# seceq/zkir

Hardware: AMD Instinct MI355X
Metric: trace rows/sec (2^20-cycle fib: execution-trace fill + BabyBear NTT/LDE + Poseidon2 Merkle commitment) (higher is better)
Workload: dtype u32 (Baby Bear, 31-bit modular) / u64 trace words

## Files before the change

### include/zkir_amd_experimental.h

```cpp
#ifndef ZKIR_AMD_EXPERIMENTAL_H
#define ZKIR_AMD_EXPERIMENTAL_H
#include "zkir_amd.h"
#ifdef __cplusplus
extern "C" {
#endif

double zkir_modmul_peak_per_s(void* hip_stream);
double zkir_hbm_copy_peak_gbs(uint64_t bytes, void* hip_stream);
int zkir_commit_fused01_launch(const zkir_stark_ctx* ctx, const zkir_trace_columns* trace, uint64_t n_real, uint32_t* m, uint32_t width, uint32_t* out, void* hip_stream);
int zkir_ntt_strided_variant_launch(const zkir_stark_ctx* ctx, uint32_t* data, uint32_t width, int variant, int forward, void* hip_stream);

int zkir_commit_overlapped_launch(const zkir_stark_ctx* ctx, uint32_t* in, uint32_t width, uint32_t* out, uint32_t* tree, uint32_t group, void* hip_stream);

int zkir_lowdeg_prove_stages(zkir_stark_ctx* ctx, const uint32_t* lde_mat, uint32_t width, const uint32_t* tree, uint32_t num_queries, uint32_t pow_bits, uint32_t* proof_host,
                             uint64_t cap_words, uint64_t* n_words, float stage_ms[4], void* hip_stream);
int zkir_lowdeg_combine_launch(const zkir_stark_ctx* ctx, const uint32_t* lde_mat, uint32_t width, const uint32_t gamma[4], uint32_t* gpow_scratch, uint32_t* cw, void* hip_stream);

int zkir_eval_prove_stages(zkir_stark_ctx* ctx, const uint32_t* lde_mat, uint32_t width, const uint32_t* tree, const uint32_t* points, uint32_t n_points, uint32_t num_queries,
                           uint32_t pow_bits, uint32_t* proof_host, uint64_t cap_words, uint64_t* n_words, float stage_ms[6], void* hip_stream);
uint64_t zkir_eval_at_scratch_words(uint32_t log_n, uint32_t width, uint32_t n_points);
int zkir_eval_at_launch(const zkir_stark_ctx* ctx, const uint32_t* lde_mat, uint32_t width, const uint32_t* points, uint32_t n_points, uint32_t* scratch, uint32_t* evals, void* hip_stream);
uint64_t zkir_eval_quotient_scratch_words(uint32_t log_m, uint32_t width, uint32_t n_points);
int zkir_eval_quotient_launch(const zkir_stark_ctx* ctx, const uint32_t* lde_mat, uint32_t width, const uint32_t gamma[4], const uint32_t* points, uint32_t n_points,
                              const uint32_t* evals, uint32_t* scratch, uint32_t* cw, void* hip_stream);
// ... 16 lines not shown
int zkir_pcs_verify_last_stage_ms(double ms[3]);
int zkir_verify_queries_last_stage_ms(double ms[3]);
int zkir_stark_query_stage_probe(const uint32_t* proof, uint64_t proof_words, uint32_t what, uint32_t index, int device, void* hip_stream);
int zkir_verify_many_memory_host(const uint32_t* const* proofs, const uint64_t* proof_words, const zkir_public_inputs* const* expects, uint32_t n, int32_t* verdicts);
int zkir_verify_rate_many_memory_host(const uint32_t* const* proofs, const uint64_t* proof_words, const zkir_public_inputs* const* expects, const uint32_t* min_queries,
                                      const uint32_t* min_pow_bits, uint32_t n, int32_t* verdicts);
int zkir_mem_sections_stage_host(const uint32_t* const* secs, const uint64_t* n_words, const uint32_t* modes, const uint64_t* code_words, const uint8_t* const* blobs, const size_t* blob_lens,
                                 const uint32_t* alphas, const uint32_t* lambdas, uint32_t n, int32_t* verdicts, uint32_t* digests, uint32_t* sums);
int zkir_mem_sections_stage_launch(const uint32_t* const* secs, const uint64_t* n_words, const uint32_t* modes, const uint64_t* code_words, const uint8_t* const* blobs, const size_t* blob_lens,
                                   const uint32_t* alphas, const uint32_t* lambdas, uint32_t n, int32_t* verdicts, uint32_t* digests, uint32_t* sums, void* hip_stream);
int zkir_verify_many_memory_probe(const uint32_t* const* proofs, const uint64_t* proof_words, const zkir_public_inputs* const* expects, uint32_t n, int32_t* verdicts, uint32_t what,
                                  uint32_t index, int device, void* hip_stream);
int zkir_verify_many_tapes_host(const uint32_t* const* proofs, const uint64_t* proof_words, const zkir_public_inputs* const* expects, uint32_t n, int32_t* verdicts);
int zkir_verify_rate_many_tapes_host(const uint32_t* const* proofs, const uint64_t* proof_words, const zkir_public_inputs* const* expects, const uint32_t* min_queries,
                                     const uint32_t* min_pow_bits, uint32_t n, int32_t* verdicts);
int zkir_tape_sections_stage_host(const uint32_t* const* hash_secs, const uint64_t* hash_words, const uint32_t* const* wide_secs, const uint64_t* wide_words, const uint64_t* n_real,
                                  const uint64_t* code_end, const uint32_t* alphas, const uint32_t* lambdas, uint32_t n, int32_t* hash_verdicts, int32_t* wide_verdicts, uint32_t* digests,
                                  uint32_t* sums);
int zkir_tape_sections_stage_launch(const uint32_t* const* hash_secs, const uint64_t* hash_words, const uint32_t* const* wide_secs, const uint64_t* wide_words, const uint64_t* n_real,
                                    const uint64_t* code_end, const uint32_t* alphas, const uint32_t* lambdas, uint32_t n, int32_t* hash_verdicts, int32_t* wide_verdicts, uint32_t* digests,
                                    uint32_t* sums, void* hip_stream);
int zkir_verify_many_tapes_probe(const uint32_t* const* proofs, const uint64_t* proof_words, const zkir_public_inputs* const* expects, uint32_t n, int32_t* verdicts, uint32_t what,
                                 uint32_t index, int device, void* hip_stream);

#ifdef __cplusplus
}
#endif
#endif
```

### zkir_amd/csrc/poseidon2.h

```cpp
#pragma once
#include "babybear.h"

#ifndef P2_RF_UNROLL
#define P2_RF_UNROLL 1
#endif
namespace p2 {

constexpr int T = 12, RF = 8, RP = 22, RATE = 8, DIGEST = 4;

struct Consts {
  uint32_t ext[RF][T];
  uint32_t in[RP];
  uint32_t diag[T];
  uint32_t pre[RF][T];
  uint32_t ext0_s[T];
  uint64_t pre_b[RF][T];
  uint32_t in_scale;
  uint32_t out_scale;
  uint32_t carry;
  int32_t in0_neg;
  int32_t pr_c[RP];
  uint64_t pr_a[RP];
  uint64_t pr_k[T];
};

inline uint64_t splitmix64(uint64_t& s) {
  uint64_t z = (s += 0x9E3779B97F4A7C15ull);
  z = (z ^ (z >> 30)) * 0xBF58476D1CE4E5B9ull;
  z = (z ^ (z >> 27)) * 0x94D049BB133111EBull;
  return z ^ (z >> 31);
}

inline void ext_matrix_inverse(uint32_t inv[T][T]) {
  static const uint32_t M4[4][4] = {{5, 7, 1, 3}, {4, 6, 1, 1}, {1, 3, 5, 7}, {1, 1, 4, 6}};
  uint32_t a[T][2 * T];
  for (int i = 0; i < T; i++)
    for (int j = 0; j < T; j++) {
      a[i][j] = M4[i & 3][j & 3] * ((i >> 2) == (j >> 2) ? 2u : 1u);
      a[i][T + j] = i == j;
    }
  for (int col = 0; col < T; col++) {
    int piv = col;
    while (a[piv][col] == 0) piv++;
    for (int j = 0; j < 2 * T; j++) { const uint32_t t = a[col][j]; a[col][j] = a[piv][j]; a[piv][j] = t; }
    const uint32_t pinv = bb::inv(a[col][col]);
    for (int j = 0; j < 2 * T; j++) a[col][j] = bb::mul(a[col][j], pinv);
    for (int i = 0; i < T; i++) {
      if (i == col || a[i][col] == 0) continue;
      const uint32_t f = a[i][col];
      for (int j = 0; j < 2 * T; j++) a[i][j] = bb::sub(a[i][j], bb::mul(f, a[col][j]));
    }
  }
  for (int i = 0; i < T; i++) for (int j = 0; j < T; j++) inv[i][j] = a[i][T + j];
}

inline void generate(Consts& c) {
  uint64_t s = 0x5A4B49522D50322Dull;
  auto next = [&]() -> uint32_t { for (;;) { const uint32_t v = (uint32_t)(splitmix64(s) >> 33); if (v < bb::P) return bb::to_mont(v); } };
  for (int r = 0; r < RF; r++) for (int i = 0; i < T; i++) c.ext[r][i] = next();
  for (int r = 0; r < RP; r++) c.in[r] = next();
  c.diag[0] = bb::to_mont(bb::P - 2);
  for (int i = 1; i < T; i++) c.diag[i] = bb::to_mont(1u << (i - 1));
  uint32_t minv[T][T];
  ext_matrix_inverse(minv);
  for (int r = 0; r < RF; r++)
    for (int i = 0; i < T; i++) {
      uint32_t v = 0;
      if (r != RF / 2 - 1 && r != RF - 1)
        for (int j = 0; j < T; j++) v = bb::add(v, bb::mul(minv[i][j], bb::from_mont(c.ext[r + 1][j])));
      c.pre[r][i] = bb::to_mont(bb::to_mont(v));
    }
  {
    constexpr uint64_t INV7 = 1725656503ull;
    const uint32_t R = bb::R1, Rinv = bb::inv(R);
    const uint32_t R6 = bb::pow(R, 6);
    uint32_t g[RF + 1], h[RF];
    g[RF / 2] = R;
    for (int r = RF / 2 - 1; r >= 0; r--) { h[r] = bb::mul(g[r + 1], R); g[r] = bb::pow(bb::mul(h[r], R6), INV7); }
    {
      uint32_t f[RP], hx[RP];
      for (int r = 0; r < RP; r++) { f[r] = r < 3 ? R : bb::mul(f[r - 3], Rinv); hx[r] = bb::pow(bb::mul(f[r], R6), INV7); }
      const uint32_t G = bb::mul(f[RP - 1], Rinv), R2c = bb::mul(R, R);
      for (int r = 0; r < RP; r++) {
        const uint32_t hn = r + 1 < RP ? hx[r + 1] : G, rcn = bb::from_mont(r + 1 < RP ? c.in[r + 1] : c.ext[RF / 2][0]);
        c.pr_c[r] = (int32_t)bb::mul(bb::mul(hn, R2c), bb::inv(f[r]));
        c.pr_a[r] = bb::mul(bb::mul(hn, rcn), R);
      }
      c.pr_k[0] = 0;
      for (int i = 1; i < T; i++) c.pr_k[i] = bb::mul(f[RP - 1], bb::from_mont(c.ext[RF / 2][i]));
      g[RF / 2] = G;
    }
    for (int r = RF / 2; r < RF; r++) { h[r] = bb::mul(bb::pow(g[r], 7), bb::inv(R6)); g[r + 1] = bb::mul(h[r], Rinv); }
    const uint32_t f_in = bb::mul(g[0], R), f_out = g[RF];
    for (int i = 0; i < T; i++) c.ext0_s[i] = bb::mul(bb::from_mont(c.ext[0][i]), f_in);
    for (int r = 0; r < RF; r++)
      for (int i = 0; i < T; i++) {
        uint32_t v = 0;
        if (r != RF / 2 - 1 && r != RF - 1)
          for (int j = 0; j < T; j++) v = bb::add(v, bb::mul(minv[i][j], bb::from_mont(c.ext[r + 1][j])));
        c.pre_b[r][i] = ((uint64_t)bb::P << 32) | bb::mul(bb::mul(v, h[r]), R);
      }
    c.in_scale = bb::mul(f_in, R);
    c.out_scale = bb::mul(R, bb::inv(f_out));
    c.carry = bb::mul(bb::mul(f_in, R), bb::inv(f_out));
// ... 114 lines not shown
  uint64_t acc = (uint64_t)w[1];
#pragma unroll
  for (int i = 2; i < T; i++) acc += (uint64_t)w[i];
  const int64_t sum = bb::sacc_add((int64_t)acc, s0);
  x = int_next_x(smad<-2>(sum, s0), c, r);
#pragma unroll
  for (int i = 1; i < T; i++) w[i] = (int64_t)(((uint64_t)w[i] << (i - 1)) + (uint64_t)sum);
}
constexpr uint64_t lazy_rounds_bound(uint64_t start, int rounds) {
  uint64_t b[T] = {}, top = 0;
  for (int i = 1; i < T; i++) b[i] = start;
  for (int r = 0; r < rounds; r++) {
    uint64_t sum = bb::P;
    for (int i = 1; i < T; i++) sum += b[i];
    if (sum + 2 * (uint64_t)bb::P > top) top = sum + 2 * (uint64_t)bb::P;
    for (int i = 1; i < T; i++) { b[i] = sum + (b[i] << (i - 1)); if (b[i] > top) top = b[i]; }
  }
  return top;
}
constexpr uint64_t lazy_reduced_bound(uint64_t acc) { return (acc >> 32) + bb::P / 2 + 2; }
static_assert(lazy_rounds_bound(1ull << 31, 3) < (1ull << 62), "three partial rounds on words below 2^31 stay inside what a Montgomery reduction takes");
static_assert(lazy_reduced_bound(lazy_rounds_bound(1ull << 31, 3)) <= (1ull << 31), ".. and their reduction is a word below 2^31 again");
static_assert(lazy_reduced_bound(lazy_rounds_bound(1ull << 31, 1) + bb::P) < bb::P, "the words leave the last round (one round + the next full round's constant) inside (-p, p)");
BB_HD void int_rounds_scaled(uint32_t* s, const Consts& c) {
  int32_t x = (int32_t)s[0] + c.in0_neg;
  int32_t t[T];
  int64_t w[T];
#pragma unroll
  for (int i = 1; i < T; i++) t[i] = (int32_t)s[i];
#pragma unroll 1
  for (int r = 0; r < RP - 1; r += 3) {
    int_round_a(x, t, w, c, r);
    int_round_w(x, w, c, r + 1);
    int_round_w(x, w, c, r + 2);
#pragma unroll
    for (int i = 1; i < T; i++) t[i] = bb::smont_reduce_wide(w[i]);
  }
  int_round_a(x, t, w, c, RP - 1);
  s[0] = (uint32_t)x;
#pragma unroll
  for (int i = 1; i < T; i++) s[i] = (uint32_t)bb::smont_reduce_wide((int64_t)((uint64_t)w[i] + c.pr_k[i]));
}
BB_HD void permute_scaled(uint32_t* s, const Consts& c) {
  ext_linear_scaled<true>(s, c.ext0_s);
#pragma unroll P2_RF_UNROLL
  for (int r = 0; r < RF / 2; r++) {
#pragma unroll
    for (int i = 0; i < T; i++) s[i] = sbox_biased(s[i], c.pre_b[r][i]);
    ext_linear_scaled<false>(s, nullptr);
  }
  int_rounds_scaled(s, c);
#pragma unroll P2_RF_UNROLL
  for (int r = RF / 2; r < RF; r++) {
#pragma unroll
    for (int i = 0; i < T; i++) s[i] = sbox_biased(s[i], c.pre_b[r][i]);
    ext_linear_scaled<false>(s, nullptr);
  }
}

#if defined(__HIPCC__)
template <int CTRL>
__device__ __forceinline__ uint32_t quad_perm(uint32_t v) { return (uint32_t)__builtin_amdgcn_mov_dpp((int)v, CTRL, 0xF, 0xF, true); }
template <int CTRL>
__device__ __forceinline__ uint64_t quad_perm64(uint64_t v) { return ((uint64_t)quad_perm<CTRL>((uint32_t)(v >> 32)) << 32) | quad_perm<CTRL>((uint32_t)v); }

template <bool ADD_RC>
__device__ __forceinline__ void ext_linear_quad_scaled(uint32_t* s, const uint32_t* m4row, const uint32_t* rc) {
  uint64_t y[3];
#pragma unroll
  for (int b = 0; b < 3; b++) {
    const uint32_t v0 = quad_perm<0x00>(s[b]), v1 = quad_perm<0x55>(s[b]), v2 = quad_perm<0xAA>(s[b]), v3 = quad_perm<0xFF>(s[b]);
    y[b] = (uint64_t)v0 * m4row[0] + (uint64_t)v1 * m4row[1] + (uint64_t)v2 * m4row[2] + (uint64_t)v3 * m4row[3];
  }
  const uint64_t sum = y[0] + y[1] + y[2];
#pragma unroll
  for (int b = 0; b < 3; b++) {
    uint64_t v = y[b] + sum;
    if (ADD_RC) v += rc[b];
    s[b] = bb::mont_reduce_wide(v);
  }
// ... 108 lines not shown
```

### zkir_amd/csrc/stark.hip

```cpp
#include <hip/hip_runtime.h>

#include <array>
#include <atomic>
#include <chrono>
#include <cstdio>
#include <cstdlib>
#include <cstddef>
#include <memory>
#include <mutex>
#include <vector>

#include "../../include/zkir_amd.h"
#include "../../include/zkir_amd_experimental.h"
#include "air.h"
#include "babybear.h"
#include "fri_shape.h"
#include "host.h"
#include "hashcall.h"
#include "poseidon2.h"
#include "verify_stages.h"

namespace {

constexpr int NT = 256;
// ... 414 lines not shown
}


__global__ __launch_bounds__(NT) void selector_inverse_kernel(uint32_t log_m, const uint32_t* __restrict__ tw_fwd, uint32_t* __restrict__ inv_xm1) {
  const uint32_t N2 = 1u << log_m, N = N2 >> 1;
  const uint32_t j0 = (blockIdx.x * NT + threadIdx.x) * 8;
  if (j0 >= N2) return;
  uint32_t d[8], pre[8];
  uint32_t run = bb::R1;
#pragma unroll
  for (int k = 0; k < 8; k++) {
    const uint32_t j = j0 + k;
    const uint32_t wj = j < N ? tw_fwd[j] : bb::neg(tw_fwd[j - N]);
    d[k] = bb::sub(bb::mont_mul(wj, bb::to_mont(bb::GEN)), bb::R1);
    pre[k] = run; run = bb::mont_mul(run, d[k]);
  }
  uint32_t inv = bb::R1, b = run, e = bb::P - 2;
  while (e) { if (e & 1) inv = bb::mont_mul(inv, b); b = bb::mont_mul(b, b); e >>= 1; }
#pragma unroll
  for (int k = 7; k >= 0; k--) { inv_xm1[j0 + k] = bb::mont_mul(inv, pre[k]); inv = bb::mont_mul(inv, d[k]); }
}


__global__ __launch_bounds__(NT) void leaf_hash_kernel(const p2::Consts* __restrict__ cp, const uint32_t* __restrict__ mat, uint32_t width, uint64_t n, uint32_t in_scale, uint32_t* __restrict__ digests) {
  const uint64_t j = (uint64_t)blockIdx.x * NT + threadIdx.x;
  if (j >= n) return;
  uint32_t s[p2::T];
#pragma unroll
  for (int i = 0; i < p2::T; i++) s[i] = 0;
  const uint4* m4 = reinterpret_cast<const uint4*>(mat);
  const uint32_t carry = cp->carry, out_scale = cp->out_scale;
  for (uint32_t off = 0; off < width; off += p2::RATE) {
    const uint4 lo = m4[((uint64_t)(off >> 3) * n + j) * 2], hi = m4[((uint64_t)(off >> 3) * n + j) * 2 + 1];
    const uint32_t v[8] = {lo.x, lo.y, lo.z, lo.w, hi.x, hi.y, hi.z, hi.w};
#pragma unroll
    for (int i = 0; i < p2::RATE; i++) s[i] = off + i < width ? bb::mont_mul_lazy(v[i], in_scale) : bb::mont_mul_lazy(s[i], carry);
#pragma unroll
    for (int i = p2::RATE; i < p2::T; i++) s[i] = bb::mont_mul_lazy(s[i], carry);
    p2::permute_scaled(s, *cp);
  }
  if (width == 0) p2::permute_scaled(s, *cp);
  uint4 d = make_uint4(bb::mont_mul(s[0], out_scale), bb::mont_mul(s[1], out_scale), bb::mont_mul(s[2], out_scale), bb::mont_mul(s[3], out_scale));
  reinterpret_cast<uint4*>(digests)[j] = d;
}

__global__ __launch_bounds__(NT) void leaf_absorb_kernel(const p2::Consts* __restrict__ cp, const uint32_t* __restrict__ mat, uint32_t width, uint32_t b0, uint32_t b1, uint64_t n, uint32_t in_scale,
                                                         uint4* __restrict__ state, int first, int last, uint32_t* __restrict__ digests) {
  const uint64_t j = (uint64_t)blockIdx.x * NT + threadIdx.x;
  if (j >= n) return;
  uint32_t s[p2::T];
  if (first) {
#pragma unroll
    for (int i = 0; i < p2::T; i++) s[i] = 0;
  } else {
    const uint4 a = state[j], b = state[n + j], c = state[2 * n + j];
    s[0] = a.x; s[1] = a.y; s[2] = a.z; s[3] = a.w; s[4] = b.x; s[5] = b.y; s[6] = b.z; s[7] = b.w; s[8] = c.x; s[9] = c.y; s[10] = c.z; s[11] = c.w;
  }
  const uint4* m4 = reinterpret_cast<const uint4*>(mat);
  const uint32_t carry = cp->carry, out_scale = cp->out_scale;
  for (uint32_t blk = b0; blk < b1; blk++) {
    const uint32_t off = blk * 8;
    const uint4 lo = m4[((uint64_t)blk * n + j) * 2], hi = m4[((uint64_t)blk * n + j) * 2 + 1];
    const uint32_t v[8] = {lo.x, lo.y, lo.z, lo.w, hi.x, hi.y, hi.z, hi.w};
#pragma unroll
    for (int i = 0; i < p2::RATE; i++) s[i] = off + i < width ? bb::mont_mul_lazy(v[i], in_scale) : bb::mont_mul_lazy(s[i], carry);
#pragma unroll
    for (int i = p2::RATE; i < p2::T; i++) s[i] = bb::mont_mul_lazy(s[i], carry);
    p2::permute_scaled(s, *cp);
  }
  if (last) {
    reinterpret_cast<uint4*>(digests)[j] = make_uint4(bb::mont_mul(s[0], out_scale), bb::mont_mul(s[1], out_scale), bb::mont_mul(s[2], out_scale), bb::mont_mul(s[3], out_scale));
  } else {
    state[j] = make_uint4(s[0], s[1], s[2], s[3]); state[n + j] = make_uint4(s[4], s[5], s[6], s[7]); state[2 * n + j] = make_uint4(s[8], s[9], s[10], s[11]);
  }
}

__global__ __launch_bounds__(NT) void compress_kernel(const p2::Consts* __restrict__ cp, const uint32_t* __restrict__ in, uint64_t n_out, uint32_t* __restrict__ out) {
  const uint64_t i = (uint64_t)blockIdx.x * NT + threadIdx.x;
  if (i >= n_out) return;
  const uint4 l = reinterpret_cast<const uint4*>(in)[2 * i], r = reinterpret_cast<const uint4*>(in)[2 * i + 1];
  const uint32_t k = cp->in_scale, ko = cp->out_scale;
  uint32_t s[p2::T] = {bb::mont_mul_lazy(l.x, k), bb::mont_mul_lazy(l.y, k), bb::mont_mul_lazy(l.z, k), bb::mont_mul_lazy(l.w, k), bb::mont_mul_lazy(r.x, k), bb::mont_mul_lazy(r.y, k),
                       bb::mont_mul_lazy(r.z, k), bb::mont_mul_lazy(r.w, k), 0, 0, 0, 0};
  p2::permute_scaled(s, *cp);
  reinterpret_cast<uint4*>(out)[i] = make_uint4(bb::mont_mul(s[0], ko), bb::mont_mul(s[1], ko), bb::mont_mul(s[2], ko), bb::mont_mul(s[3], ko));
}

constexpr uint32_t SUBTREE = 1024, NT_SUB = 1024;
__global__ __launch_bounds__(NT_SUB) void subtree_kernel(const p2::Consts* __restrict__ cp, uint32_t* cur, uint64_t m, uint32_t per_wg, uint32_t* counter) {
  __shared__ uint4 buf[SUBTREE];
  __shared__ uint32_t last_one;
  const uint32_t t = threadIdx.x;
  uint64_t pos0 = (uint64_t)blockIdx.x * per_wg;
  for (uint32_t e = t; e < per_wg; e += NT_SUB) {
    const uint4 v = reinterpret_cast<const uint4*>(cur)[pos0 + e];
    buf[e] = make_uint4(bb::to_mont(v.x), bb::to_mont(v.y), bb::to_mont(v.z), bb::to_mont(v.w));
  }
  __syncthreads();
 levels:
  for (uint32_t cnt = per_wg; cnt > 1; cnt >>= 1) {
    cur += 4 * m; m >>= 1; pos0 >>= 1;
    const uint32_t n_perm = cnt / 2;
    if (n_perm > NT_SUB / 16) {
      const bool active = t < n_perm;
      uint32_t s[p2::T];
      if (active) {
        const uint4 l = buf[2 * t], r = buf[2 * t + 1];
// ... 95 lines not shown
    hipLaunchKernelGGL(compress_kernel, dim3(grid_for(m / 2)), dim3(NT), 0, s, cp, cur, m / 2, nxt);
    cur = nxt;
  }
  if (m > 1) {
    const uint32_t per = m < SUBTREE ? (uint32_t)m : SUBTREE;
    hipLaunchKernelGGL(subtree_kernel, dim3((unsigned)(m / per)), dim3(NT_SUB), 0, s, cp, cur, m, per, ring.take());
  }
}

}

struct zkir_stark_ctx {
  uint32_t log_n = 0, log_blowup = 1;
  uint32_t* d_tw_inv = nullptr;
  uint32_t* d_tw_fwd = nullptr;
  uint32_t* d_g_lo = nullptr;
  uint32_t* d_g_lo_m = nullptr;
  mutable uint32_t* d_inv_xm1 = nullptr;
  uint32_t* d_g_hi = nullptr;
  uint32_t* d_small_inv = nullptr;
  uint32_t* d_small_fwd = nullptr;
  p2::Consts consts;
  p2::Consts* d_p2 = nullptr;
  mutable hipStream_t ov_stream = nullptr; mutable hipEvent_t ov_ev[2] = {nullptr, nullptr}; mutable std::vector<hipEvent_t> ov_group_ev; mutable uint4* d_ov_state = nullptr; mutable size_t ov_state_bytes = 0;
  mutable SyncRing sync;
  mutable ZeroFlagRing zero;
  mutable std::mutex mu;
  mutable unsigned char* arena = nullptr;
  mutable size_t arena_size = 0, arena_off = 0;
  mutable zkir::HostPin pin;
  mutable const uint32_t* rate_mats[3] = {nullptr, nullptr, nullptr};
  mutable uint32_t rate_widths[3] = {0, 0, 0};
};

namespace {
const char* const BLOWUP2_ONLY = ": the context has log_blowup != 1; the prover's quotient, DEEP and FRI stages (and the experiments built on its LDE) are blow-up 2 — contexts of log_blowup 2 / 3 serve zkir_lde_launch and the zkir_merkle_* calls";
bool blowup2_only(const zkir_stark_ctx* c, const char* who) {
  if (c->log_blowup == 1) return true;
  zkir::set_last_error({ZKIR_ERR_ARGUMENT, std::string(who) + BLOWUP2_ONLY});
  return false;
}
int lde_launch(const zkir_stark_ctx* c, uint32_t* in, uint32_t width, uint32_t* out, bool mont_out, hipStream_t s) {
  zkir::LdeTables t{(int)c->log_n, c->d_tw_inv, c->d_tw_fwd, mont_out ? c->d_g_lo_m : c->d_g_lo, c->d_g_hi, c->d_small_inv, c->d_small_fwd, (int)c->log_blowup};
  if (c->log_blowup == 1 && c->log_n >= 14) c->zero.take(t.zero_slot, t.zero_epoch);
  zkir::lde_run(t, in, (width + 7) / 8, out, s);
  return check_launch("lde");
}
int merkle_commit(const zkir_stark_ctx* c, const uint32_t* mat, uint32_t width, uint64_t n_leaves, uint32_t* tree, bool mont_in, hipStream_t s) {
  hipLaunchKernelGGL(leaf_hash_kernel, dim3(grid_for(n_leaves)), dim3(NT), 0, s, c->d_p2, mat, width, n_leaves, mont_in ? bb::from_mont(c->consts.in_scale) : c->consts.in_scale, tree);
  launch_tree_levels(c->d_p2, tree, n_leaves, c->sync, s);
  return check_launch("merkle_commit");
}
int selector_table_ensure(const zkir_stark_ctx* c, hipStream_t s) {
  if (c->d_inv_xm1) return ZKIR_OK;
  const uint64_t M = 1ull << (c->log_n + c->log_blowup);
  uint32_t* t = nullptr;
  if (hipMalloc(&t, (size_t)M * 4) != hipSuccess) { zkir::set_last_error({ZKIR_ERR_DEVICE, "zkir_prove_rate: no device memory for the selector table"}); return ZKIR_ERR_DEVICE; }
  hipLaunchKernelGGL(selector_inverse_kernel, dim3(grid_for((M + 7) / 8)), dim3(NT), 0, s, c->log_n + c->log_blowup, c->d_tw_fwd, t);
  c->d_inv_xm1 = t;
  return check_launch("selector table");
}
}

extern "C" {

uint32_t zkir_main_trace_width(void) { return air::committed_width(false); }
uint32_t zkir_main_trace_width_for(uint32_t deferred) { return air::committed_width((int)deferred); }

void zkir_poseidon2_permute(uint32_t state[12]) {
  static const p2::Consts consts = [] { p2::Consts c; p2::generate(c); return c; }();
  uint32_t s[p2::T];
  for (int i = 0; i < p2::T; i++) s[i] = bb::to_mont(state[i] % bb::P);
  p2::permute(s, consts);
  for (int i = 0; i < p2::T; i++) state[i] = bb::from_mont(s[i]);
}

void zkir_poseidon2_permute_scaled(uint32_t state[12], uint32_t rounds) {
  static const p2::Consts consts = [] { p2::Consts c; p2::generate(c); return c; }();
  uint32_t s[p2::T];
  for (int i = 0; i < p2::T; i++) s[i] = bb::mont_mul_lazy(state[i] % bb::P, consts.in_scale);
  for (uint32_t r = 0; r < rounds; r++) {
    if (r) for (int i = 0; i < p2::T; i++) s[i] = bb::mont_mul_lazy(s[i], consts.carry);
    p2::permute_scaled(s, consts);
  }
  for (int i = 0; i < p2::T; i++) state[i] = rounds ? bb::mont_mul(s[i], consts.out_scale) : state[i] % bb::P;
}

namespace { typedef uint32_t u32x4 __attribute__((ext_vector_type(4)));
__global__ __launch_bounds__(NT) void copy16_kernel(const u32x4* __restrict__ src, u32x4* __restrict__ dst, uint64_t n) {
  const uint64_t stride = (uint64_t)gridDim.x * NT;
  uint64_t i = (uint64_t)blockIdx.x * NT + threadIdx.x;
  for (; i + 3 * stride < n; i += 4 * stride) {
    const u32x4 a = __builtin_nontemporal_load(src + i), b = __builtin_nontemporal_load(src + i + stride), c = __builtin_nontemporal_load(src + i + 2 * stride), d = __builtin_nontemporal_load(src + i + 3 * stride);
    __builtin_nontemporal_store(a, dst + i); __builtin_nontemporal_store(b, dst + i + stride); __builtin_nontemporal_store(c, dst + i + 2 * stride); __builtin_nontemporal_store(d, dst + i + 3 * stride);
  }
  for (; i < n; i += stride) dst[i] = src[i];
} }
double zkir_hbm_copy_peak_gbs(uint64_t bytes, void* stream) {
  hipStream_t s = (hipStream_t)stream;
  const uint64_t n = (bytes >> 14) << 10;
  if (!n) return 0.0;
  u32x4 *a = nullptr, *b = nullptr;
  if (hipMalloc((void**)&a, n * 16) != hipSuccess) return 0.0;
  if (hipMalloc((void**)&b, n * 16) != hipSuccess) { (void)hipFree(a); return 0.0; }
  (void)hipMemsetAsync(a, 1, n * 16, s);
  hipEvent_t e0, e1;
  (void)hipEventCreate(&e0); (void)hipEventCreate(&e1);
  double best = 0.0;
// ... 26 lines not shown
  hipLaunchKernelGGL(modmul_peak_kernel, dim3(blocks), dim3(NT), 0, s, d, iters);
  (void)hipEventRecord(b, s);
  (void)hipEventSynchronize(b);
  float ms = 0;
  (void)hipEventElapsedTime(&ms, a, b);
  (void)hipEventDestroy(a); (void)hipEventDestroy(b); (void)hipFree(d);
  return ms > 0 ? (double)blocks * NT * iters * 8.0 / (ms * 1e-3) : 0.0;
}

int zkir_stark_ctx_create(uint32_t log_n, uint32_t log_blowup, zkir_stark_ctx** out) {
  if (!out || log_n < 1 || log_n > 26 || log_blowup < 1 || log_blowup > 3 || log_n + log_blowup > 27) {
    zkir::set_last_error({ZKIR_ERR_ARGUMENT, "zkir_stark_ctx_create: need 1 <= log_n <= 26, log_blowup in {1, 2, 3} and log_n + log_blowup <= 27 (the field's two-adicity)"});
    return ZKIR_ERR_ARGUMENT;
  }
  *out = nullptr;
  zkir_stark_ctx* c = new zkir_stark_ctx();
  c->log_n = log_n; c->log_blowup = log_blowup;
  const uint32_t N = 1u << log_n;
  const uint32_t n_inv = N >= 2 ? N / 2 : 1, n_hi = (N >> 10) + 1;
  const uint32_t n_fwd = N << (log_blowup - 1);
  p2::generate(c->consts);
  hipError_t e = hipMalloc((void**)&c->d_p2, sizeof(p2::Consts));
  if (e == hipSuccess) e = hipMemcpy(c->d_p2, &c->consts, sizeof(p2::Consts), hipMemcpyHostToDevice);
  if (e == hipSuccess) e = hipMalloc(&c->sync.d_slots, SYNC_SLOTS * sizeof(uint32_t));
  if (e == hipSuccess) e = hipMemset(c->sync.d_slots, 0, SYNC_SLOTS * sizeof(uint32_t));
  if (e == hipSuccess) e = hipMalloc(&c->zero.d_words, (size_t)ZERO_SLOTS * zkir::ZERO_FLAG_BLOCKS * sizeof(uint32_t));
  if (e == hipSuccess) e = hipMemset(c->zero.d_words, 0, (size_t)ZERO_SLOTS * zkir::ZERO_FLAG_BLOCKS * sizeof(uint32_t));
  if (e == hipSuccess) e = hipMalloc(&c->d_tw_inv, (size_t)n_inv * 4);
  if (e == hipSuccess) e = hipMalloc(&c->d_tw_fwd, (size_t)n_fwd * 4);
  if (e == hipSuccess) e = hipMalloc(&c->d_g_lo, 1024 * 4);
  if (e == hipSuccess) e = hipMalloc(&c->d_g_hi, (size_t)n_hi * 4);
  if (e == hipSuccess) e = hipMalloc(&c->d_g_lo_m, 1024 * 4);
  if (e == hipSuccess && log_blowup == 1) e = hipMalloc(&c->d_inv_xm1, (size_t)2 * N * 4);
  const int Bm = log_n < 10 ? (int)log_n : 10;
  const uint32_t n_si = Bm >= 1 ? (1u << (Bm - 1)) : 1, n_sf = 1u << (Bm + log_blowup - 1);
  if (e == hipSuccess) e = hipMalloc(&c->d_small_inv, (size_t)n_si * 4);
  if (e == hipSuccess) e = hipMalloc(&c->d_small_fwd, (size_t)n_sf * 4);
  if (e != hipSuccess) { zkir::set_last_error({ZKIR_ERR_DEVICE, std::string("zkir_stark_ctx_create: ") + hipGetErrorString(e)}); zkir_stark_ctx_free(c); return ZKIR_ERR_DEVICE; }
  const uint32_t wN = bb::root_of_unity(log_n), wM = bb::root_of_unity(log_n + log_blowup);
  hipLaunchKernelGGL(powers_kernel, dim3(grid_for(n_inv)), dim3(NT), 0, 0, bb::inv(wN), bb::R1, c->d_tw_inv, n_inv);
  hipLaunchKernelGGL(powers_kernel, dim3(grid_for(n_fwd)), dim3(NT), 0, 0, wM, bb::R1, c->d_tw_fwd, n_fwd);
  hipLaunchKernelGGL(powers_kernel, dim3(4), dim3(NT), 0, 0, bb::GEN, bb::to_mont(bb::inv(N % bb::P)), c->d_g_lo, 1024u);
  hipLaunchKernelGGL(powers_kernel, dim3(4), dim3(NT), 0, 0, bb::GEN, bb::to_mont(bb::to_mont(bb::inv(N % bb::P))), c->d_g_lo_m, 1024u);
  hipLaunchKernelGGL(powers_kernel, dim3(grid_for(n_hi)), dim3(NT), 0, 0, bb::pow(bb::GEN, 1024), bb::R1, c->d_g_hi, n_hi);
  if (log_blowup == 1) hipLaunchKernelGGL(selector_inverse_kernel, dim3(grid_for((2ull * N + 7) / 8)), dim3(NT), 0, 0, log_n + 1, c->d_tw_fwd, c->d_inv_xm1);
  hipLaunchKernelGGL(powers_kernel, dim3(grid_for(n_si)), dim3(NT), 0, 0, bb::inv(bb::root_of_unity(Bm)), bb::R1, c->d_small_inv, n_si);
  hipLaunchKernelGGL(powers_kernel, dim3(grid_for(n_sf)), dim3(NT), 0, 0, bb::root_of_unity(Bm + log_blowup), bb::R1, c->d_small_fwd, n_sf);
  if (hipDeviceSynchronize() != hipSuccess || check_launch("stark ctx tables") != ZKIR_OK) { zkir_stark_ctx_free(c); return ZKIR_ERR_DEVICE; }
  *out = c;
  return ZKIR_OK;
}

void zkir_stark_ctx_free(zkir_stark_ctx* c) {
  if (!c) return;
  (void)hipFree(c->d_tw_inv); (void)hipFree(c->d_tw_fwd); (void)hipFree(c->d_g_lo); (void)hipFree(c->d_g_hi); (void)hipFree(c->d_g_lo_m); (void)hipFree(c->d_inv_xm1);
  (void)hipFree(c->d_small_inv); (void)hipFree(c->d_small_fwd); (void)hipFree(c->d_p2); (void)hipFree(c->sync.d_slots); (void)hipFree(c->zero.d_words);
  if (c->ov_stream) (void)hipStreamDestroy(c->ov_stream);
  for (hipEvent_t e : c->ov_ev) if (e) (void)hipEventDestroy(e);
  for (hipEvent_t e : c->ov_group_ev) (void)hipEventDestroy(e);
  (void)hipFree(c->d_ov_state);
  if (c->arena) (void)hipFree(c->arena);
  delete c;
}

uint32_t zkir_stark_ctx_log_blowup(const zkir_stark_ctx* c) { return c ? c->log_blowup : 0; }

uint32_t zkir_padded_log_n(uint64_t n_real) { uint32_t k = 3; while (((uint64_t)1 << k) < n_real) k++; return k; }

int zkir_main_trace_launch(const zkir_trace_columns* trace, uint64_t n_real, uint32_t deferred, uint32_t* out, void* stream) {
  if (!trace || !out || n_real == 0 || deferred > 1) { zkir::set_last_error({ZKIR_ERR_ARGUMENT, "zkir_main_trace_launch: null argument, empty trace, or a mode other than 0 / 1 (mode 2: zkir_main_trace_io_launch)"}); return ZKIR_ERR_ARGUMENT; }
  const uint64_t N = (uint64_t)1 << zkir_padded_log_n(n_real);
  if (deferred) hipLaunchKernelGGL(main_trace_kernel<1>, dim3(grid_for(N)), dim3(NT), 0, (hipStream_t)stream, *trace, n_real, N, out, IoRowArgs{});
  else hipLaunchKernelGGL(main_trace_kernel<0>, dim3(grid_for(N)), dim3(NT), 0, (hipStream_t)stream, *trace, n_real, N, out, IoRowArgs{});
  return check_launch("main_trace");
}
int zkir_main_trace_io_launch(const zkir_trace_columns* trace, uint64_t n_real, const zkir_io_args* io, uint32_t* scratch, uint32_t* out, void* stream) {
  if (!trace || !out || !io || !scratch || n_real == 0 || (!io->inputs && io->n_inputs)) { zkir::set_last_error({ZKIR_ERR_ARGUMENT, "zkir_main_trace_io_launch: null argument or empty trace"}); return ZKIR_ERR_ARGUMENT; }
  hipStream_t s = (hipStream_t)stream;
  const uint64_t N = (uint64_t)1 << zkir_padded_log_n(n_real);
// ... 111 lines not shown
  const zkir::LdeTables t{(int)c->log_n, c->d_tw_inv, c->d_tw_fwd, c->d_g_lo, c->d_g_hi, c->d_small_inv, c->d_small_fwd};
  (void)hipEventRecord(c->ov_ev[0], s); (void)hipStreamWaitEvent(c->ov_stream, c->ov_ev[0], 0);
  for (uint32_t g = 0; g < n_groups; g++) {
    const uint32_t b0 = g * group, b1 = std::min(nb, b0 + group);
    zkir::lde_run(t, in + (uint64_t)b0 * N * 8, b1 - b0, out + (uint64_t)b0 * N2 * 8, s);
    (void)hipEventRecord(c->ov_group_ev[g], s); (void)hipStreamWaitEvent(c->ov_stream, c->ov_group_ev[g], 0);
    hipLaunchKernelGGL(leaf_absorb_kernel, dim3(grid_for(N2)), dim3(NT), 0, c->ov_stream, c->d_p2, out, width, b0, b1, N2, c->consts.in_scale, c->d_ov_state, g == 0 ? 1 : 0, g + 1 == n_groups ? 1 : 0, tree);
  }
  (void)hipEventRecord(c->ov_ev[1], c->ov_stream); (void)hipStreamWaitEvent(s, c->ov_ev[1], 0);
  launch_tree_levels(c->d_p2, tree, N2, c->sync, s);
  return check_launch("commit_overlapped");
}

int zkir_lde_launch(const zkir_stark_ctx* c, uint32_t* in, uint32_t width, uint32_t* out, void* stream) { return lde_launch(c, in, width, out, false, (hipStream_t)stream); }

int zkir_merkle_commit_launch(const zkir_stark_ctx* c, const uint32_t* mat, uint32_t width, uint64_t n_leaves, uint32_t* tree, void* stream) {
  hipStream_t s = (hipStream_t)stream;
  if (!c || n_leaves == 0 || (n_leaves & (n_leaves - 1))) { zkir::set_last_error({ZKIR_ERR_ARGUMENT, "merkle: null context, or n_leaves not a power of two"}); return ZKIR_ERR_ARGUMENT; }
  return merkle_commit(c, mat, width, n_leaves, tree, false, s);
}

int zkir_merkle_leaves_launch(const zkir_stark_ctx* c, const uint32_t* mat, uint32_t width, uint64_t n_leaves, uint32_t* digests, void* stream) {
  if (!c || !mat || !digests || n_leaves == 0) { zkir::set_last_error({ZKIR_ERR_ARGUMENT, "merkle leaves: null argument or no leaves"}); return ZKIR_ERR_ARGUMENT; }
  hipLaunchKernelGGL(leaf_hash_kernel, dim3(grid_for(n_leaves)), dim3(NT), 0, (hipStream_t)stream, c->d_p2, mat, width, n_leaves, c->consts.in_scale, digests);
  return check_launch("merkle_leaves");
}

int zkir_merkle_cap_launch(const zkir_stark_ctx* c, uint32_t* tree, uint64_t n_digests, void* stream) {
  if (!c || n_digests == 0 || (n_digests & (n_digests - 1))) { zkir::set_last_error({ZKIR_ERR_ARGUMENT, "merkle cap: null context, or n_digests not a power of two"}); return ZKIR_ERR_ARGUMENT; }
  launch_tree_levels(c->d_p2, tree, n_digests, c->sync, (hipStream_t)stream);
  return check_launch("merkle_cap");
}

}

#include "fri.inl"
#include "stark_prove.inl"
#include "merkle_open.inl"
#include "lowdeg.inl"
#include "eval_open.inl"
#include "mixed_eval.inl"
#include "query_stage.inl"
#include "pcs_verify.inl"
#include "mixed_verify.inl"
#include "stark_verify.inl"
#include "pcs_verify_many.inl"
```

### zkir_amd/runtime.py

```python
from __future__ import annotations

import ctypes as C
import os
from dataclasses import dataclass
from typing import List, Optional, Sequence, Tuple

import numpy as np

from .spec import Program

_HERE = os.path.dirname(os.path.abspath(__file__))
_SO = os.environ.get("ZKIR_AMD_LIB") or os.path.join(_HERE, "libzkir_amd.so")

(ZKIR_OK, ERR_MISALIGNED, ERR_INVALID_MEMORY, ERR_DIV_ZERO, ERR_INVALID_SYSCALL, ERR_DECODE, ERR_OTHER, ERR_BAD_PROGRAM,
 ERR_DEVICE, ERR_ARGUMENT) = range(10)
HALT_EBREAK, HALT_EXIT, HALT_CYCLE_LIMIT = 0, 1, 2

REG_EVENT_DTYPE = np.dtype([("value", "<u8"), ("payload", "<u8"), ("max_bits", "<u4"), ("vis", "<u4"), ("reg", "u1"),
                            ("state", "u1"), ("tag", "u1"), ("pad", "u1", (5,))])
MEM_EVENT_DTYPE = np.dtype([("address", "<u8"), ("value", "<u8"), ("row", "<u4"), ("is_write", "u1"), ("width", "u1"), ("pad", "<u2")])
RC_EVENT_DTYPE = np.dtype([("value", "<u8"), ("pc", "<u8")])
NORM_EVENT_DTYPE = np.dtype([("cycle", "<u8"), ("pc", "<u8"), ("raw_value", "<u8"), ("reg", "u1"), ("state", "u1"), ("opcode", "u1"),
                             ("pad", "u1", (5,))])
SHA_BLOCK_DTYPE = np.dtype([("message_block", "<u4", (16,)), ("timestamp", "<u8")])
# ... 412 lines not shown
        L.zkir_verify_rate_device.restype = C.c_int; L.zkir_verify_rate_device.argtypes = [V, U64, C.POINTER(PublicInputsC), U32, U32, V]
        L.zkir_prove_rate_last_matrices.restype = C.c_int; L.zkir_prove_rate_last_matrices.argtypes = [V, V, V, V, V, C.POINTER(U64)]
    if hasattr(L, "zkir_prove_rate_modes"):
        L.zkir_prove_rate_modes.restype = C.c_int; L.zkir_prove_rate_modes.argtypes = L.zkir_prove_rate.argtypes
        L.zkir_prove_result_rate.restype = C.c_int
        L.zkir_prove_result_rate.argtypes = [V, C.POINTER(ProverParamsC), U32, C.POINTER(C.POINTER(C.c_uint8)), C.POINTER(C.c_size_t)]
    if hasattr(L, "zkir_prove_rate_segment"):
        L.zkir_prove_rate_segment.restype = C.c_int; L.zkir_prove_rate_segment.argtypes = L.zkir_prove_rate.argtypes
        L.zkir_verify_rate_segment.restype = C.c_int; L.zkir_verify_rate_segment.argtypes = [V, U64, C.POINTER(PublicInputsC), U32, U32, V, V]
        L.zkir_verify_rate_chain.restype = C.c_int; L.zkir_verify_rate_chain.argtypes = [V, V, U32, C.POINTER(PublicInputsC), U32, U32]
        L.zkir_verify_rate_segment_device.restype = C.c_int; L.zkir_verify_rate_segment_device.argtypes = [V, U64, C.POINTER(PublicInputsC), U32, U32, V, V, V]
        L.zkir_verify_rate_chain_device.restype = C.c_int; L.zkir_verify_rate_chain_device.argtypes = [V, V, U32, C.POINTER(PublicInputsC), U32, U32, V]
        L.zkir_verify_rate_many_device.restype = C.c_int; L.zkir_verify_rate_many_device.argtypes = [V, V, V, V, V, U32, V, V]
        L.zkir_pcs_verify_many_device.restype = C.c_int; L.zkir_pcs_verify_many_device.argtypes = [V, V, V, V, V, V, U32, V, V]
    L.zkir_prove_result.restype = C.c_int
    L.zkir_prove_result.argtypes = [V, C.POINTER(ProverParamsC), C.POINTER(C.POINTER(C.c_uint8)), C.POINTER(C.c_size_t)]
    L.zkir_proof_bytes_free.restype = None
    L.zkir_proof_bytes_free.argtypes = [C.POINTER(C.c_uint8)]
    L.zkir_proof_free.restype = None
    L.zkir_proof_free.argtypes = [C.POINTER(C.c_uint32)]
    L.zkir_proof_num_queries.restype = U32
    L.zkir_poseidon2_permute.restype = None; L.zkir_poseidon2_permute.argtypes = [C.c_void_p]
    L.zkir_poseidon2_permute_scaled.restype = None; L.zkir_poseidon2_permute_scaled.argtypes = [C.c_void_p, C.c_uint32]
    L.zkir_exec.restype = C.c_int
    L.zkir_exec.argtypes = [C.c_char_p, C.c_size_t, C.POINTER(C.c_uint64), C.c_size_t, C.POINTER(VmConfigC), C.POINTER(C.c_void_p)]
    L.zkir_result_free.argtypes = [C.c_void_p]
    L.zkir_result_free.restype = None
    L.zkir_result_delta_log.restype = C.c_void_p
    L.zkir_result_delta_log.argtypes = [C.c_void_p]
    L.zkir_result_trace.restype = C.POINTER(TraceColumnsC)
    L.zkir_result_trace.argtypes = [C.c_void_p]
    L.zkir_result_stage_ms.restype = None
    L.zkir_result_stage_ms.argtypes = [C.c_void_p, C.POINTER(C.c_float)]
    L.zkir_result_copy_column.restype = C.c_int
    L.zkir_result_copy_column.argtypes = [C.c_void_p, C.c_int, C.c_int, C.c_void_p]
    for name, st in [("memory_trace", MemoryWitnessC), ("range_check_witnesses", RangeCheckWitnessC),
                     ("normalization_witnesses", NormalizationWitnessC), ("sha256_witnesses", Sha256WitnessC)]:
        f = getattr(L, "zkir_result_" + name)
        f.restype = C.c_int
        f.argtypes = [C.c_void_p, C.POINTER(st)]
    L.zkir_host_to_device.restype = C.c_int
    L.zkir_host_to_device.argtypes = [C.c_void_p, C.c_void_p, C.c_size_t, C.c_void_p]
    L.zkir_device_to_host.restype = C.c_int
    L.zkir_device_to_host.argtypes = [C.c_void_p, C.c_void_p, C.c_size_t]
    _lib = L
    return L
# ... 870 lines not shown
```

Before: 204.5 million.

## Trim Poseidon2 leaf/node hashing: partial last linear layer, folded input scaling

Leaf hashing for widths that are a multiple of the rate now runs through a new full-block sponge. It skips the per-word input Montgomery scaling by folding that scale into a second, forward-form constant set, with a generate() variant that sets the first S-box scale. The last permutation's external linear layer now computes only the quad actually consumed: the capacity quad between blocks and the digest quad at the end. Tree-node compression does the same through permute_scaled_quad<0>. This removes multiplies from the hash-heavy Merkle commit, at the cost of extra constant tables, a kernel specialization, and tighter lazy-reduction bounds checked by static_asserts.

```diff
diff --git a/include/zkir_amd_experimental.h b/include/zkir_amd_experimental.h
--- a/include/zkir_amd_experimental.h
+++ b/include/zkir_amd_experimental.h
@@ -62,6 +62,8 @@
                                     uint32_t* sums, void* hip_stream);
 int zkir_verify_many_tapes_probe(const uint32_t* const* proofs, const uint64_t* proof_words, const zkir_public_inputs* const* expects, uint32_t n, int32_t* verdicts, uint32_t what,
                                  uint32_t index, int device, void* hip_stream);
+void zkir_poseidon2_scaled_quads(const uint32_t* in, uint64_t n, uint32_t* full, uint32_t* quads);
+int zkir_poseidon2_sponge_full_blocks(const uint32_t* words, uint32_t n_words, uint32_t form, uint32_t digest[4]);
 
 #ifdef __cplusplus
 }
diff --git a/zkir_amd/csrc/poseidon2.h b/zkir_amd/csrc/poseidon2.h
--- a/zkir_amd/csrc/poseidon2.h
+++ b/zkir_amd/csrc/poseidon2.h
@@ -22,6 +22,8 @@
   int32_t pr_c[RP];
   uint64_t pr_a[RP];
   uint64_t pr_k[T];
+  int32_t pr_c0;
+  uint64_t pr_a0;
 };
 
 inline uint64_t splitmix64(uint64_t& s) {
@@ -54,7 +56,7 @@
   for (int i = 0; i < T; i++) for (int j = 0; j < T; j++) inv[i][j] = a[i][T + j];
 }
 
-inline void generate(Consts& c) {
+inline void generate(Consts& c, uint32_t f0 = 0) {
   uint64_t s = 0x5A4B49522D50322Dull;
   auto next = [&]() -> uint32_t { for (;;) { const uint32_t v = (uint32_t)(splitmix64(s) >> 33); if (v < bb::P) return bb::to_mont(v); } };
   for (int r = 0; r < RF; r++) for (int i = 0; i < T; i++) c.ext[r][i] = next();
@@ -75,11 +77,19 @@
     const uint32_t R = bb::R1, Rinv = bb::inv(R);
     const uint32_t R6 = bb::pow(R, 6);
     uint32_t g[RF + 1], h[RF];
-    g[RF / 2] = R;
-    for (int r = RF / 2 - 1; r >= 0; r--) { h[r] = bb::mul(g[r + 1], R); g[r] = bb::pow(bb::mul(h[r], R6), INV7); }
+    if (f0 == 0) {
+      g[RF / 2] = R;
+      for (int r = RF / 2 - 1; r >= 0; r--) { h[r] = bb::mul(g[r + 1], R); g[r] = bb::pow(bb::mul(h[r], R6), INV7); }
+    } else {
+      g[0] = bb::mul(f0 % bb::P, Rinv);
+      for (int r = 0; r < RF / 2; r++) { h[r] = bb::mul(bb::pow(g[r], 7), bb::inv(R6)); g[r + 1] = bb::mul(h[r], Rinv); }
+    }
     {
+      const uint32_t F = g[RF / 2];
       uint32_t f[RP], hx[RP];
-      for (int r = 0; r < RP; r++) { f[r] = r < 3 ? R : bb::mul(f[r - 3], Rinv); hx[r] = bb::pow(bb::mul(f[r], R6), INV7); }
+      for (int r = 0; r < RP; r++) { f[r] = r < 3 ? F : bb::mul(f[r - 3], Rinv); hx[r] = bb::pow(bb::mul(f[r], R6), INV7); }
+      c.pr_c0 = (int32_t)bb::mul(bb::mul(hx[0], R), bb::inv(F));
+      c.pr_a0 = bb::mul(bb::mul(hx[0], bb::from_mont(c.in[0])), R);
       const uint32_t G = bb::mul(f[RP - 1], Rinv), R2c = bb::mul(R, R);
       for (int r = 0; r < RP; r++) {
         const uint32_t hn = r + 1 < RP ? hx[r + 1] : G, rcn = bb::from_mont(r + 1 < RP ? c.in[r + 1] : c.ext[RF / 2][0]);
@@ -240,8 +250,10 @@
 static_assert(lazy_rounds_bound(1ull << 31, 3) < (1ull << 62), "three partial rounds on words below 2^31 stay inside what a Montgomery reduction takes");
 static_assert(lazy_reduced_bound(lazy_rounds_bound(1ull << 31, 3)) <= (1ull << 31), ".. and their reduction is a word below 2^31 again");
 static_assert(lazy_reduced_bound(lazy_rounds_bound(1ull << 31, 1) + bb::P) < bb::P, "the words leave the last round (one round + the next full round's constant) inside (-p, p)");
+static_assert((((uint64_t)bb::P + 128) * bb::P >> 32) + 2 + bb::P / 2 < bb::P, "word 0 enters its first S-box inside (-p, p)");
+template <bool ENTRY = false>
 BB_HD void int_rounds_scaled(uint32_t* s, const Consts& c) {
-  int32_t x = (int32_t)s[0] + c.in0_neg;
+  int32_t x = ENTRY ? bb::smont_mul_add((int32_t)s[0], c.pr_c0, c.pr_a0) : (int32_t)s[0] + c.in0_neg;
   int32_t t[T];
   int64_t w[T];
 #pragma unroll
@@ -274,6 +286,77 @@
     for (int i = 0; i < T; i++) s[i] = sbox_biased(s[i], c.pre_b[r][i]);
     ext_linear_scaled<false>(s, nullptr);
   }
+}
+
+constexpr uint64_t EXT_IN_MAX = (uint64_t)bb::P * 196 / 100 + 1;
+static_assert(4 * EXT_IN_MAX < (1ull << 34), "u_j, the sum of a column's three words with one counted twice, is below 2^34");
+static_assert(16 * 4 * EXT_IN_MAX < (1ull << 38), "M4's rows sum to at most 16: every output is below 2^38 before its reduction, as in ext_linear_scaled");
+static_assert(((16 * 4 * EXT_IN_MAX) >> 32) + bb::P < bb::P + 64, ".. and leaves it below p + 64");
+BB_HD void m4_wide64(uint64_t a, uint64_t b, uint64_t c, uint64_t d, uint64_t* y) {
+  const uint64_t t0 = a + b, t1 = c + d;
+  const uint64_t t2 = (b << 1) + t1, t3 = (d << 1) + t0;
+  const uint64_t t4 = (t1 << 2) + t3, t5 = (t0 << 2) + t2;
+  y[0] = t3 + t5; y[1] = t5; y[2] = t2 + t4; y[3] = t4;
+}
+template <int Q>
+BB_HD void ext_linear_scaled_quad(const uint32_t* s, uint32_t* out4) {
+  static_assert(Q >= 0 && Q < 3, "a state has three quads");
+  constexpr int A = Q == 0 ? 1 : 0, B = Q == 2 ? 1 : 2;
+  uint64_t u[4], y[4];
+#pragma unroll
+  for (int j = 0; j < 4; j++) u[j] = bb::acc_add(bb::mad_wide<2>((uint64_t)s[4 * A + j], s[4 * Q + j]), s[4 * B + j]);
+  m4_wide64(u[0], u[1], u[2], u[3], y);
+#pragma unroll
+  for (int j = 0; j < 4; j++) out4[j] = bb::mont_reduce_wide(y[j]);
+}
+template <bool ENTRY = false>
+BB_HD void permute_scaled_head(uint32_t* s, const Consts& c) {
+  ext_linear_scaled<true>(s, c.ext0_s);
+#pragma unroll P2_RF_UNROLL
+  for (int r = 0; r < RF / 2; r++) {
+#pragma unroll
+    for (int i = 0; i < T; i++) s[i] = sbox_biased(s[i], c.pre_b[r][i]);
+    ext_linear_scaled<false>(s, nullptr);
+  }
+  int_rounds_scaled<ENTRY>(s, c);
+#pragma unroll P2_RF_UNROLL
+  for (int r = RF / 2; r < RF - 1; r++) {
+#pragma unroll
+    for (int i = 0; i < T; i++) s[i] = sbox_biased(s[i], c.pre_b[r][i]);
+    ext_linear_scaled<false>(s, nullptr);
+  }
+  int r_last = RF - 1;
+#if defined(__HIP_DEVICE_COMPILE__)
+  asm volatile("" : "+s"(r_last));
+#endif
+#pragma unroll
+  for (int i = 0; i < T; i++) s[i] = sbox_biased(s[i], c.pre_b[r_last][i]);
+}
+template <int Q, bool ENTRY = false>
+BB_HD void permute_scaled_quad(uint32_t* s, const Consts& c) {
+  permute_scaled_head<ENTRY>(s, c);
+  ext_linear_scaled_quad<Q>(s, s + 4 * Q);
+}
+static_assert(16 * (4 * 0xFFFFFFFFull) < (1ull << 38) && ((16 * (4 * 0xFFFFFFFFull) + bb::P) >> 32) + bb::P < bb::P + 128, "the initial layer takes absorbed words of any value");
+template <bool FORWARD, class Load>
+BB_HD void sponge_full_blocks(Load&& load, uint32_t n_blocks, uint32_t in_scale, const Consts& c, uint32_t* digest4) {
+  uint32_t s[T];
+#pragma unroll
+  for (int i = RATE; i < T; i++) s[i] = 0;
+  for (uint32_t b = 0;;) {
+    uint32_t v[RATE];
+    load(b, v);
+#pragma unroll
+    for (int i = 0; i < RATE; i++) s[i] = FORWARD ? v[i] : bb::mont_mul_lazy(v[i], in_scale);
+    permute_scaled_head<FORWARD>(s, c);
+    if (++b == n_blocks) break;
+    ext_linear_scaled_quad<2>(s, s + 8);
+#pragma unroll
+    for (int i = RATE; i < T; i++) s[i] = bb::mont_mul_lazy(s[i], c.carry);
+  }
+  ext_linear_scaled_quad<0>(s, s);
+#pragma unroll
+  for (int i = 0; i < DIGEST; i++) digest4[i] = bb::mont_mul(s[i], c.out_scale);
 }
 
 #if defined(__HIPCC__)
diff --git a/zkir_amd/csrc/stark.hip b/zkir_amd/csrc/stark.hip
--- a/zkir_amd/csrc/stark.hip
+++ b/zkir_amd/csrc/stark.hip
@@ -460,10 +460,22 @@
 }
 
 
-__global__ __launch_bounds__(NT) void leaf_hash_kernel(const p2::Consts* __restrict__ cp, const uint32_t* __restrict__ mat, uint32_t width, uint64_t n, uint32_t in_scale, uint32_t* __restrict__ digests) {
+constexpr bool LEAF_FORWARD = true;
+template <bool FULL_BLOCKS>
+__device__ __forceinline__ void leaf_hash_body(const p2::Consts* __restrict__ cp, const uint32_t* __restrict__ mat, uint32_t width, uint64_t n, uint32_t in_scale, uint32_t* __restrict__ digests) {
   const uint64_t j = (uint64_t)blockIdx.x * NT + threadIdx.x;
   if (j >= n) return;
   uint32_t s[p2::T];
+  if constexpr (FULL_BLOCKS) {
+    const uint4* m4 = reinterpret_cast<const uint4*>(mat) + 2 * j;
+    uint32_t d[p2::DIGEST];
+    p2::sponge_full_blocks<LEAF_FORWARD>([&](uint32_t blk, uint32_t* v) {
+      const uint4 lo = m4[(uint64_t)blk * n * 2], hi = m4[(uint64_t)blk * n * 2 + 1];
+      v[0] = lo.x; v[1] = lo.y; v[2] = lo.z; v[3] = lo.w; v[4] = hi.x; v[5] = hi.y; v[6] = hi.z; v[7] = hi.w;
+    }, width >> 3, in_scale, *cp, d);
+    reinterpret_cast<uint4*>(digests)[j] = make_uint4(d[0], d[1], d[2], d[3]);
+    return;
+  }
 #pragma unroll
   for (int i = 0; i < p2::T; i++) s[i] = 0;
   const uint4* m4 = reinterpret_cast<const uint4*>(mat);
@@ -480,6 +492,16 @@
   if (width == 0) p2::permute_scaled(s, *cp);
   uint4 d = make_uint4(bb::mont_mul(s[0], out_scale), bb::mont_mul(s[1], out_scale), bb::mont_mul(s[2], out_scale), bb::mont_mul(s[3], out_scale));
   reinterpret_cast<uint4*>(digests)[j] = d;
+}
+__global__ __launch_bounds__(NT) void leaf_hash_kernel(const p2::Consts* __restrict__ cp, const uint32_t* __restrict__ mat, uint32_t width, uint64_t n, uint32_t in_scale, uint32_t* __restrict__ digests) {
+  leaf_hash_body<true>(cp, mat, width, n, in_scale, digests);
+}
+__global__ __launch_bounds__(NT) void leaf_hash_ragged_kernel(const p2::Consts* __restrict__ cp, const uint32_t* __restrict__ mat, uint32_t width, uint64_t n, uint32_t in_scale, uint32_t* __restrict__ digests) {
+  leaf_hash_body<false>(cp, mat, width, n, in_scale, digests);
+}
+void leaf_hash_launch(const p2::Consts* cp, const p2::Consts* cp_fwd, const uint32_t* mat, uint32_t width, uint64_t n, uint32_t in_scale, uint32_t* digests, hipStream_t s) {
+  if (width != 0 && width % p2::RATE == 0) hipLaunchKernelGGL(leaf_hash_kernel, dim3(grid_for(n)), dim3(NT), 0, s, LEAF_FORWARD ? cp_fwd : cp, mat, width, n, in_scale, digests);
+  else hipLaunchKernelGGL(leaf_hash_ragged_kernel, dim3(grid_for(n)), dim3(NT), 0, s, cp, mat, width, n, in_scale, digests);
 }
 
 __global__ __launch_bounds__(NT) void leaf_absorb_kernel(const p2::Consts* __restrict__ cp, const uint32_t* __restrict__ mat, uint32_t width, uint32_t b0, uint32_t b1, uint64_t n, uint32_t in_scale,
@@ -520,7 +542,7 @@
   const uint32_t k = cp->in_scale, ko = cp->out_scale;
   uint32_t s[p2::T] = {bb::mont_mul_lazy(l.x, k), bb::mont_mul_lazy(l.y, k), bb::mont_mul_lazy(l.z, k), bb::mont_mul_lazy(l.w, k), bb::mont_mul_lazy(r.x, k), bb::mont_mul_lazy(r.y, k),
                        bb::mont_mul_lazy(r.z, k), bb::mont_mul_lazy(r.w, k), 0, 0, 0, 0};
-  p2::permute_scaled(s, *cp);
+  p2::permute_scaled_quad<0>(s, *cp);
   reinterpret_cast<uint4*>(out)[i] = make_uint4(bb::mont_mul(s[0], ko), bb::mont_mul(s[1], ko), bb::mont_mul(s[2], ko), bb::mont_mul(s[3], ko));
 }
 
@@ -662,6 +684,7 @@
   uint32_t* d_small_fwd = nullptr;
   p2::Consts consts;
   p2::Consts* d_p2 = nullptr;
+  p2::Consts* d_p2_fwd[2] = {nullptr, nullptr};
   mutable hipStream_t ov_stream = nullptr; mutable hipEvent_t ov_ev[2] = {nullptr, nullptr}; mutable std::vector<hipEvent_t> ov_group_ev; mutable uint4* d_ov_state = nullptr; mutable size_t ov_state_bytes = 0;
   mutable SyncRing sync;
   mutable ZeroFlagRing zero;
@@ -687,7 +710,7 @@
   return check_launch("lde");
 }
 int merkle_commit(const zkir_stark_ctx* c, const uint32_t* mat, uint32_t width, uint64_t n_leaves, uint32_t* tree, bool mont_in, hipStream_t s) {
-  hipLaunchKernelGGL(leaf_hash_kernel, dim3(grid_for(n_leaves)), dim3(NT), 0, s, c->d_p2, mat, width, n_leaves, mont_in ? bb::from_mont(c->consts.in_scale) : c->consts.in_scale, tree);
+  leaf_hash_launch(c->d_p2, c->d_p2_fwd[mont_in ? 1 : 0], mat, width, n_leaves, mont_in ? bb::from_mont(c->consts.in_scale) : c->consts.in_scale, tree, s);
   launch_tree_levels(c->d_p2, tree, n_leaves, c->sync, s);
   return check_launch("merkle_commit");
 }
@@ -724,6 +747,33 @@
     p2::permute_scaled(s, consts);
   }
   for (int i = 0; i < p2::T; i++) state[i] = rounds ? bb::mont_mul(s[i], consts.out_scale) : state[i] % bb::P;
+}
+
+void zkir_poseidon2_scaled_quads(const uint32_t* in, uint64_t n, uint32_t* full, uint32_t* quads) {
+  static const p2::Consts consts = [] { p2::Consts c; p2::generate(c); return c; }();
+  for (uint64_t k = 0; k < n; k++) {
+    uint32_t s[p2::T], q[p2::T];
+    for (int i = 0; i < p2::T; i++) s[i] = in[12 * k + i];
+    p2::permute_scaled(s, consts);
+    for (int i = 0; i < p2::T; i++) full[12 * k + i] = s[i];
+    for (int i = 0; i < p2::T; i++) q[i] = in[12 * k + i];
+    p2::permute_scaled_quad<0>(q, consts);
+    for (int j = 0; j < 4; j++) quads[12 * k + j] = q[j];
+    for (int i = 0; i < p2::T; i++) q[i] = in[12 * k + i];
+    p2::permute_scaled_quad<1>(q, consts);
+    for (int j = 0; j < 4; j++) quads[12 * k + 4 + j] = q[4 + j];
+    for (int i = 0; i < p2::T; i++) q[i] = in[12 * k + i];
+    p2::permute_scaled_quad<2>(q, consts);
+    for (int j = 0; j < 4; j++) quads[12 * k + 8 + j] = q[8 + j];
+  }
+}
+int zkir_poseidon2_sponge_full_blocks(const uint32_t* words, uint32_t n_words, uint32_t form, uint32_t digest[4]) {
+  if (!words || !digest || n_words == 0 || n_words % p2::RATE != 0 || form > 2) { zkir::set_last_error({ZKIR_ERR_ARGUMENT, "zkir_poseidon2_sponge_full_blocks: need a non-zero multiple of 8 words and form 0 / 1 / 2"}); return ZKIR_ERR_ARGUMENT; }
+  static const p2::Consts consts[3] = {[] { p2::Consts c; p2::generate(c); return c; }(), [] { p2::Consts c; p2::generate(c, 1u); return c; }(), [] { p2::Consts c; p2::generate(c, bb::R1); return c; }()};
+  const auto load = [&](uint32_t b, uint32_t* v) { for (int i = 0; i < p2::RATE; i++) v[i] = words[8 * b + i]; };
+  if (form == 0) p2::sponge_full_blocks<false>(load, n_words / p2::RATE, consts[0].in_scale, consts[0], digest);
+  else p2::sponge_full_blocks<true>(load, n_words / p2::RATE, 0, consts[form], digest);
+  return ZKIR_OK;
 }
 
 namespace { typedef uint32_t u32x4 __attribute__((ext_vector_type(4)));
@@ -796,6 +846,12 @@
   p2::generate(c->consts);
   hipError_t e = hipMalloc((void**)&c->d_p2, sizeof(p2::Consts));
   if (e == hipSuccess) e = hipMemcpy(c->d_p2, &c->consts, sizeof(p2::Consts), hipMemcpyHostToDevice);
+  for (int m = 0; m < 2 && e == hipSuccess; m++) {
+    p2::Consts fwd;
+    p2::generate(fwd, m ? bb::R1 : 1u);
+    e = hipMalloc((void**)&c->d_p2_fwd[m], sizeof(p2::Consts));
+    if (e == hipSuccess) e = hipMemcpy(c->d_p2_fwd[m], &fwd, sizeof(p2::Consts), hipMemcpyHostToDevice);
+  }
   if (e == hipSuccess) e = hipMalloc(&c->sync.d_slots, SYNC_SLOTS * sizeof(uint32_t));
   if (e == hipSuccess) e = hipMemset(c->sync.d_slots, 0, SYNC_SLOTS * sizeof(uint32_t));
   if (e == hipSuccess) e = hipMalloc(&c->zero.d_words, (size_t)ZERO_SLOTS * zkir::ZERO_FLAG_BLOCKS * sizeof(uint32_t));
@@ -828,7 +884,7 @@
 void zkir_stark_ctx_free(zkir_stark_ctx* c) {
   if (!c) return;
   (void)hipFree(c->d_tw_inv); (void)hipFree(c->d_tw_fwd); (void)hipFree(c->d_g_lo); (void)hipFree(c->d_g_hi); (void)hipFree(c->d_g_lo_m); (void)hipFree(c->d_inv_xm1);
-  (void)hipFree(c->d_small_inv); (void)hipFree(c->d_small_fwd); (void)hipFree(c->d_p2); (void)hipFree(c->sync.d_slots); (void)hipFree(c->zero.d_words);
+  (void)hipFree(c->d_small_inv); (void)hipFree(c->d_small_fwd); (void)hipFree(c->d_p2); (void)hipFree(c->d_p2_fwd[0]); (void)hipFree(c->d_p2_fwd[1]); (void)hipFree(c->sync.d_slots); (void)hipFree(c->zero.d_words);
   if (c->ov_stream) (void)hipStreamDestroy(c->ov_stream);
   for (hipEvent_t e : c->ov_ev) if (e) (void)hipEventDestroy(e);
   for (hipEvent_t e : c->ov_group_ev) (void)hipEventDestroy(e);
@@ -986,7 +1042,7 @@
 
 int zkir_merkle_leaves_launch(const zkir_stark_ctx* c, const uint32_t* mat, uint32_t width, uint64_t n_leaves, uint32_t* digests, void* stream) {
   if (!c || !mat || !digests || n_leaves == 0) { zkir::set_last_error({ZKIR_ERR_ARGUMENT, "merkle leaves: null argument or no leaves"}); return ZKIR_ERR_ARGUMENT; }
-  hipLaunchKernelGGL(leaf_hash_kernel, dim3(grid_for(n_leaves)), dim3(NT), 0, (hipStream_t)stream, c->d_p2, mat, width, n_leaves, c->consts.in_scale, digests);
+  leaf_hash_launch(c->d_p2, c->d_p2_fwd[0], mat, width, n_leaves, c->consts.in_scale, digests, (hipStream_t)stream);
   return check_launch("merkle_leaves");
 }
 
diff --git a/zkir_amd/runtime.py b/zkir_amd/runtime.py
--- a/zkir_amd/runtime.py
+++ b/zkir_amd/runtime.py
@@ -458,6 +458,9 @@
     L.zkir_proof_num_queries.restype = U32
     L.zkir_poseidon2_permute.restype = None; L.zkir_poseidon2_permute.argtypes = [C.c_void_p]
     L.zkir_poseidon2_permute_scaled.restype = None; L.zkir_poseidon2_permute_scaled.argtypes = [C.c_void_p, C.c_uint32]
+    if hasattr(L, "zkir_poseidon2_scaled_quads"):
+        L.zkir_poseidon2_scaled_quads.restype = None; L.zkir_poseidon2_scaled_quads.argtypes = [C.c_void_p, C.c_uint64, C.c_void_p, C.c_void_p]
+        L.zkir_poseidon2_sponge_full_blocks.restype = C.c_int; L.zkir_poseidon2_sponge_full_blocks.argtypes = [C.c_void_p, C.c_uint32, C.c_uint32, C.c_void_p]
     L.zkir_exec.restype = C.c_int
     L.zkir_exec.argtypes = [C.c_char_p, C.c_size_t, C.POINTER(C.c_uint64), C.c_size_t, C.POINTER(VmConfigC), C.POINTER(C.c_void_p)]
     L.zkir_result_free.argtypes = [C.c_void_p]
```

Result: faster. 208.7 million, median of 6 (+2.1%).
